# husheng876/pytorch_nested-unet

Hardware: AMD Instinct MI355X
Metric: images/sec NestedUNet 96x96 bs=16 train (higher is better)
Workload: dtype bf16; 1 GPU; NestedUNet(num_classes=1, in=3, deep_supervision=False) 96x96 per-GPU batch 16, bf16 storage / fp32 accumulate, BCEDiceLoss, SGD(1e-3, 0.9, wd 1e-4), fwd+loss+iou+bwd+sgd per step (BASELINE.json configs[1]); global_batch=16, parallelism=dp1, hip_graph=True

## Files before the change

include/nunet.h:

```cpp
#ifndef NUNET_H
#define NUNET_H

#include <stddef.h>
#include <stdint.h>

#ifdef __cplusplus
extern "C" {
#endif

typedef void* nunet_stream_t;

enum { NUNET_F32 = 0, NUNET_BF16 = 1, NUNET_F16 = 2 };
enum {
  NUNET_OK = 0,
  NUNET_EINVAL = -1,
  NUNET_ELAUNCH = -2,
  NUNET_ENODEV = -3
};

int nunet_version(void);
const char* nunet_last_error(void);

#define NUNET_BN_SUM_REPLICAS 8
#define NUNET_FX_WORDS 2

enum { NUNET_TF_NONE = 0, NUNET_TF_BN_RELU = 1, NUNET_TF_BN_RELU_BWD = 2 };

typedef struct {
  int32_t dtype;
  int32_t N, H, W;
  const void* src0; int32_t C0, P0;
  const void* src1; int32_t C1, P1;
  const void* wpack;
  const float* bias;
  void* dst0; int32_t D0, Q0;
  void* dst1; int32_t D1, Q1;
  int32_t acc_slot_w;
  uint32_t acc0_mask;
  int32_t acc1;
  int64_t* stats;
  float* splitk_ws;
  int64_t splitk_ws_floats;
  const void* bn_y; int32_t bn_py;
  const float* bn_mean_invstd;
  const float* bn_gamma; const float* bn_beta;
  int64_t* bn_sums;
  int32_t in_tf;
  int32_t tf_training;
  const void* tf_y; int32_t tf_py;
  const int64_t* tf_fx;
  const float* tf_gamma; const float* tf_beta; const float* tf_conv_bias;
  float* tf_running_mean; float* tf_running_var; int64_t* tf_nbt;
  float* tf_mean_invstd;
  float tf_momentum, tf_eps;
  float* tf_dgamma; float* tf_dbeta; float* tf_dbias;
  void* tf_store; int32_t tf_ps;
  int32_t tile;
} nunet_conv_desc;

int nunet_conv3x3_fwd(const nunet_conv_desc* d, nunet_stream_t s);

typedef struct {
  int32_t dtype;
  int32_t N, H, W;
  const void* src0; int32_t C0, P0;
  const void* src1; int32_t C1, P1;
  const void* dy;   int32_t Cout, PY;
  float* dw;
  int64_t slab_stride;
  int32_t max_slabs;
  int32_t target_wgs;
  int64_t dw_floats;
  int32_t item_shape;
} nunet_wgrad_desc;

int32_t nunet_conv3x3_wgrad_slabs(const nunet_wgrad_desc* d);
int nunet_conv3x3_wgrad(const nunet_wgrad_desc* d, nunet_stream_t s);
int nunet_conv3x3_wgrad_pair(const nunet_wgrad_desc* a, const nunet_wgrad_desc* b, nunet_stream_t stream);
int nunet_wgrad_reduce(const float* slabs, int64_t slab_stride, int32_t nslabs, int64_t n, float* out,
                       int32_t accumulate, nunet_stream_t s);

int nunet_pack_weights(const float* w_oihw, int32_t cout, int32_t cin, int32_t cin_pad,
                       int32_t dtype, void* wf, void* wd, nunet_stream_t s);
int nunet_unpack_wgrad(const float* dw, int32_t cout, int32_t cin, int32_t cin_pad,
                       float* g_oihw, int32_t accumulate, nunet_stream_t s);

typedef struct {
  int32_t dtype;
  int32_t N, H, W, C;
  const void* y; int32_t PY;
// ... 195 lines not shown
```

pytorch_nested-unet_amd/_lib.py:

```python
import ctypes as C
import os
import subprocess

import torch

_HERE = os.path.dirname(os.path.abspath(__file__))
LIB_PATH = os.environ.get("NUNET_LIB_PATH") or os.path.join(_HERE, "libnunet.so")

F32, BF16, F16 = 0, 1, 2
DTYPES = {"fp32": F32, "float32": F32, "bf16": BF16, "bfloat16": BF16, "fp16": F16, "float16": F16,
          torch.float32: F32, torch.bfloat16: BF16, torch.float16: F16}
TORCH_DTYPE = {F32: torch.float32, BF16: torch.bfloat16, F16: torch.float16}

_vp, _i32, _i64, _u32, _f32, _sz = C.c_void_p, C.c_int32, C.c_int64, C.c_uint32, C.c_float, C.c_size_t
BN_SUM_REPLICAS = 8
FX_WORDS = 2
TF_NONE, TF_BN_RELU, TF_BN_RELU_BWD = 0, 1, 2


def fx_zeros(c, device):
    return torch.zeros(BN_SUM_REPLICAS * 2 * c * FX_WORDS, dtype=torch.int64, device=device)


def fx_decode(buf, c):
    w = buf.detach().cpu().view(BN_SUM_REPLICAS, 2 * c, FX_WORDS).sum(0)
    return w[:, 0].double() * 2.0 ** -20 + w[:, 1].double() * 2.0 ** -60


def fx_encode(values, c, device):
    v = values.detach().cpu().double().reshape(2 * c) * 2.0 ** 20
    hi = torch.floor(v)
    lo = torch.floor((v - hi) * 2.0 ** 40)
    buf = torch.zeros(BN_SUM_REPLICAS, 2 * c, FX_WORDS, dtype=torch.int64)
    buf[0, :, 0] = hi.to(torch.int64)
    buf[0, :, 1] = lo.to(torch.int64)
    return buf.reshape(-1).to(device)


class ConvDesc(C.Structure):
    _fields_ = [("dtype", _i32), ("N", _i32), ("H", _i32), ("W", _i32),
                ("src0", _vp), ("C0", _i32), ("P0", _i32),
                ("src1", _vp), ("C1", _i32), ("P1", _i32),
                ("wpack", _vp), ("bias", _vp),
                ("dst0", _vp), ("D0", _i32), ("Q0", _i32),
                ("dst1", _vp), ("D1", _i32), ("Q1", _i32),
                ("acc_slot_w", _i32), ("acc0_mask", _u32), ("acc1", _i32),
                ("stats", _vp), ("splitk_ws", _vp), ("splitk_ws_floats", _i64),
                ("bn_y", _vp), ("bn_py", _i32), ("bn_mean_invstd", _vp), ("bn_gamma", _vp), ("bn_beta", _vp), ("bn_sums", _vp),
                ("in_tf", _i32), ("tf_training", _i32), ("tf_y", _vp), ("tf_py", _i32), ("tf_fx", _vp),
                ("tf_gamma", _vp), ("tf_beta", _vp), ("tf_conv_bias", _vp),
                ("tf_running_mean", _vp), ("tf_running_var", _vp), ("tf_nbt", _vp), ("tf_mean_invstd", _vp),
                ("tf_momentum", _f32), ("tf_eps", _f32),
                ("tf_dgamma", _vp), ("tf_dbeta", _vp), ("tf_dbias", _vp), ("tf_store", _vp), ("tf_ps", _i32), ("tile", _i32)]


class WgradDesc(C.Structure):
    _fields_ = [("dtype", _i32), ("N", _i32), ("H", _i32), ("W", _i32),
                ("src0", _vp), ("C0", _i32), ("P0", _i32),
                ("src1", _vp), ("C1", _i32), ("P1", _i32),
                ("dy", _vp), ("Cout", _i32), ("PY", _i32),
                ("dw", _vp), ("slab_stride", _i64), ("max_slabs", _i32), ("target_wgs", _i32), ("dw_floats", _i64), ("item_shape", _i32)]


class BnFwdDesc(C.Structure):
    _fields_ = [("dtype", _i32), ("N", _i32), ("H", _i32), ("W", _i32), ("C", _i32),
                ("y", _vp), ("PY", _i32),
                ("conv_bias", _vp), ("stats", _vp), ("gamma", _vp), ("beta", _vp),
                ("running_mean", _vp), ("running_var", _vp), ("num_batches_tracked", _vp),
                ("save_mean_invstd", _vp),
                ("training", _i32), ("momentum", _f32), ("eps", _f32),
                ("a", _vp), ("PA", _i32), ("pooled", _vp), ("PP", _i32), ("up", _vp), ("PU", _i32)]


class BnBwdDesc(C.Structure):
    _fields_ = [("dtype", _i32), ("N", _i32), ("H", _i32), ("W", _i32), ("C", _i32),
                ("da", _vp), ("PDA", _i32), ("y", _vp), ("PY", _i32),
                ("mean_invstd", _vp), ("gamma", _vp), ("beta", _vp),
                ("sums", _vp), ("dgamma", _vp), ("dbeta", _vp), ("dbias", _vp),
                ("dy", _vp), ("PDY", _i32)]


class BnrDesc(C.Structure):
    _fields_ = [("y", _vp), ("PY", _i32), ("mean_invstd", _vp), ("gamma", _vp), ("beta", _vp), ("sums", _vp)]


class ProfEntry(C.Structure):
# ... 180 lines not shown
```

pytorch_nested-unet_amd/csrc/conv3x3.hip:

```cpp
#include <stdlib.h>
#include <type_traits>

#include "common.h"

template <typename T> struct Mma;
template <> struct Mma<bf16_t> {
  typedef bf16x8 Frag;
  static __device__ __forceinline__ Frag load(const bf16_t* p) { return *reinterpret_cast<const bf16x8*>(p); }
  static __device__ __forceinline__ void mma(f32x16& acc, const Frag& a, const Frag& b) {
    acc = __builtin_amdgcn_mfma_f32_32x32x16_bf16(a, b, acc, 0, 0, 0);
  }
  static __device__ __forceinline__ void sink(const Frag& a) { asm volatile("" :: "v"(a)); }
};
template <> struct Mma<f16_t> {
  typedef f16x8 Frag;
  static __device__ __forceinline__ Frag load(const f16_t* p) { return *reinterpret_cast<const f16x8*>(p); }
  static __device__ __forceinline__ void mma(f32x16& acc, const Frag& a, const Frag& b) {
    acc = __builtin_amdgcn_mfma_f32_32x32x16_f16(a, b, acc, 0, 0, 0);
  }
  static __device__ __forceinline__ void sink(const Frag& a) { asm volatile("" :: "v"(a)); }
};
template <> struct Mma<float> {
  struct Frag { f32x4 lo, hi; };
  static __device__ __forceinline__ Frag load(const float* p) {
// ... 28 lines not shown
}

__host__ __device__ __forceinline__ unsigned fastdiv_inv(int d) { return d > 1 ? (unsigned)(((1ull << 32) + (unsigned)d - 1) / (unsigned)d) : 0u; }
__device__ __forceinline__ int fastdiv(int n, unsigned inv) { return inv ? (int)__umulhi((unsigned)n, inv) : n; }

template <bool ST>
__device__ __forceinline__ int map_pixel_t(int n, int y, int x, int N, int H, int W, int SH, unsigned SHinv) {
  if constexpr (ST) {
    const int yc = y < 0 ? 0 : y;
    const int n2 = (int)__umulhi((unsigned)yc, SHinv), yy = yc - n2 * SH - 1;
    const bool ok = (y >= 0) & (x >= 0) & (x < W) & (n2 < N) & (yy >= 0);
    const int gp = (n2 * H + yy) * W + x;
    return ok ? gp : -1;
  } else {
    const bool ok = (n < N) & (y >= 0) & (y < H) & (x >= 0) & (x < W);
    const int gp = (n * H + y) * W + x;
    return ok ? gp : -1;
  }
}

__device__ __attribute__((aligned(64))) uint32_t g_zero_page[2048 + 16];

struct ConvP {
  const void* src0; const void* src1;
  int C0, C1, P0, P1;
  const void* w; const float* bias;
  void* dst0; void* dst1;
  int D0, D1, Q0, Q1;
  int slot_w; unsigned acc0_mask; int acc1;
  unsigned inv_slot_w;
  long long* stats;
  int N, H, W, Cin, Cout;
  int NI, TH, TW, tilesX, tilesY, tilesG, nCoT, nItems;
  int SH;
  unsigned SHinv;
  unsigned invS, invCoT, invTX, invTY;
  unsigned invTHW, invTW, invHH2HW2, invHW2;
  int S, nch0, nch;
  float* slabs;
  long long slab_stride;
  const void* bn_y; int bn_py;
  const float* bn_mi; const float* bn_gamma; const float* bn_beta;
  long long* bn_sums;
  const void* tf_y; int tf_py;
  const long long* tf_fx;
  const float* tf_gamma; const float* tf_beta; const float* tf_bias;
  float* tf_rm; float* tf_rv; long long* tf_nbt;
  float* tf_save;
  int tf_training; float tf_momentum, tf_eps;
  float* tf_dgamma; float* tf_dbeta; float* tf_dbias;
  void* tf_store; int tf_ps;
  float M;
};

template <typename T, int WM_, int WN_, int SM_, int SN_> struct ConvCfg {
  static constexpr int WM = WM_, WN = WN_, SM = SM_, SN = SN_;
  static constexpr int NT = 64 * WM * WN;
  static constexpr int BM = 32 * SM * WM;
  static constexpr int BN = 32 * SN * WN;
  static constexpr int EPV = Tr<T>::EPV;
  static constexpr int KC = 64 / (int)sizeof(T);
  static constexpr int KS = KC / 16;
  static constexpr int PS = KC + EPV;
  static constexpr int HPMAX = (SM * SN == 4) ? 344 : BM + BM / 2;
  static constexpr int UH = (HPMAX * 4 + NT - 1) / NT;
  static constexpr int UW = (9 * BN * 4 + NT - 1) / NT;
  static constexpr int OS = BN + EPV;
  static constexpr int UO = (BM * (BN / EPV) + NT - 1) / NT;
  static constexpr int HALO_ELEMS = HPMAX * PS;
  static constexpr int W_ELEMS = 9 * BN * PS;
  static constexpr int STAGE_ELEMS = (HALO_ELEMS + W_ELEMS) > BM * OS ? (HALO_ELEMS + W_ELEMS) : BM * OS;
};

#ifdef NUNET_KSTAMP
__device__ unsigned long long* g_kstamp; __device__ int g_kstamp_wgs;
extern "C" int nunet_kstamp_set(void* buf, int wgs) {
  if (hipMemcpyToSymbol(HIP_SYMBOL(g_kstamp), &buf, sizeof(buf)) != hipSuccess) return 1;
  return hipMemcpyToSymbol(HIP_SYMBOL(g_kstamp_wgs), &wgs, sizeof(wgs)) != hipSuccess;
}
#define KSTAMP(i) do { if (threadIdx.x == 0 && (int)blockIdx.x < g_kstamp_wgs && (i) < 30) g_kstamp[blockIdx.x * 32 + (i)] = __builtin_amdgcn_s_memtime(); } while (0)
#define KSTAMP_RT(i) do { if (threadIdx.x == 0 && (int)blockIdx.x < g_kstamp_wgs) g_kstamp[blockIdx.x * 32 + (i)] = __builtin_amdgcn_s_memrealtime(); } while (0)
#else
#define KSTAMP(i) do {} while (0)
#define KSTAMP_RT(i) do {} while (0)
#endif

#ifndef NUNET_ABLATE
#define NUNET_ABLATE 0
#endif

static inline int conv_coef_floats(int lt, int cin, bool bnr, int cout) { return (lt == 1 ? 2 : lt == 2 ? 4 : 0) * cin + (bnr ? 4 * cout : 0) + cout; }

struct ConvGroup { int n; int grid[CONV_GROUP_MAX]; ConvP p[CONV_GROUP_MAX]; };

#ifndef NUNET_XCD_REMAP
#define NUNET_XCD_REMAP 1
#endif
__device__ __forceinline__ int xcd_remap(int b, int G) {
  if (!NUNET_XCD_REMAP) return b;
  const int x = b & 7, l = b >> 3, q = G >> 3, rem = G & 7;
  return (x < rem ? x * (q + 1) : rem * (q + 1) + (x - rem) * q) + l;
}
__device__ __forceinline__ void conv_group_decode(const ConvGroup& g, int b, int& k, int& v) {
  int base = 0, prevg = 0, live = g.n;
  k = 0; v = b;
#pragma unroll
  for (int j = 0; j < CONV_GROUP_MAX; ++j) {
    if (j < g.n) {
      const int span = (g.grid[j] - prevg) * live;
      if (b >= base && b < base + span) { const int r = b - base; const int q = r / live; k = j + (r - q * live); v = prevg + q; }
      base += span; prevg = g.grid[j]; --live;
    }
  }
}

template <typename T, int WM, int WN, int SM, int SN, bool SK, bool BNR, int LT>
__global__ __launch_bounds__(64 * WM * WN, 2) void conv3x3_kernel(ConvGroup grp) {
  typedef ConvCfg<T, WM, WN, SM, SN> C;
  int gk = 0, vbid = (int)blockIdx.x;
  if (grp.n > 1) conv_group_decode(grp, (int)blockIdx.x, gk, vbid);
  gk = __builtin_amdgcn_readfirstlane(gk); vbid = __builtin_amdgcn_readfirstlane(vbid);
  const ConvP& p = grp.p[gk];
  const int vgrid = grp.grid[gk];
  typedef Mma<T> M;
  constexpr int PS = C::PS, EPV = C::EPV, BN = C::BN, BM = C::BM, NT = C::NT, KS = C::KS, OS = C::OS;

  __shared__ __attribute__((aligned(16))) T s_buf[C::STAGE_ELEMS];
  __shared__ int s_hidx[BM];
  __shared__ int s_mxy[BM];
  __shared__ int s_hxy[C::HPMAX];
  __shared__ int s_gpix[BM];
  __shared__ float s_red[2 * WM * BN];
  extern __shared__ __attribute__((aligned(16))) float s_coef[];
  T* const s_halo = s_buf;
  T* const s_w = s_buf + C::HALO_ELEMS;
  float* const s_bnc = s_coef + (LT == 1 ? 2 : LT == 2 ? 4 : 0) * p.Cin;
  float* const s_bias = s_bnc + (BNR ? 4 : 0) * p.Cout;

  const int tid = threadIdx.x, lane = tid & 63, wave = tid >> 6;
  const int wm = wave / WN, wn = wave % WN;
  const int r = lane & 31, h = lane >> 5;
  const int HW2 = p.TW + 2, HH2 = p.TH + 2;
  const int HP = p.NI * HH2 * HW2;
  const int THW = p.TH * p.TW;
  KSTAMP(0); KSTAMP_RT(30);
  [[maybe_unused]] int kst = 4;

  for (int m = tid; m < BM; m += NT) {
    const int r32 = m & 31;
    const int q = (r32 < 4) ? r32 : (r32 < 12) ? r32 + 12 : (r32 < 16) ? r32 - 8 : (r32 < 20) ? r32 + 8 : (r32 < 28) ? r32 - 12 : r32;
    const int t = (m & ~31) + q;
    const int ni = fastdiv(t, p.invTHW);
    const int rem = t - ni * THW;
    const int ly = fastdiv(rem, p.invTW), lx = rem - ly * p.TW;
    const bool ok = ni < p.NI;
    s_hidx[m] = ok ? ((ni * HH2 + ly + 1) * HW2 + lx + 1) : (HW2 + 1);
    s_mxy[m] = ok ? ((ni << 20) | (ly << 10) | lx) : -1;
  }
  for (int hp = tid; hp < C::HPMAX; hp += NT) {
    int code = -1;
    if (hp < HP) {
      const int ni = fastdiv(hp, p.invHH2HW2);
      const int rem = hp - ni * (HH2 * HW2);
      const int hy = fastdiv(rem, p.invHW2), hx = rem - hy * HW2;
      code = (ni << 20) | (hy << 10) | hx;
    }
    s_hxy[hp] = code;
  }
// ... 58 lines not shown
    const int row = u >> 2;
    const int tap = row / BN, co = row - tap * BN;
    woff[k] = row < 9 * BN ? (unsigned)(((tap * p.Cout + co) * p.Cin + seg * EPV) * (int)sizeof(T)) : (unsigned)(seg * 16);
  }
  unsigned wco = 0u;
  auto set_ptrs = [&](const Item& it) { wco = (unsigned)(it.co0 * p.Cin * (int)sizeof(T)); };
  struct LoadCtx { const char* base; unsigned pb, cb, yb, ycb, wb; };
  auto load_ctx = [&](int kb) {
    LoadCtx c;
    const bool s0 = LT != 0 || kb < p.C0;
    c.base = (const char*)(s0 ? p.src0 : p.src1);
    c.pb = (unsigned)(s0 ? p.P0 : p.P1) * (unsigned)sizeof(T);
    c.cb = (unsigned)((s0 ? kb : kb - p.C0) * (int)sizeof(T) + seg * 16);
    c.yb = (unsigned)p.tf_py * (unsigned)sizeof(T);
    c.ycb = (unsigned)(kb * (int)sizeof(T) + seg * 16);
    c.wb = (unsigned)(kb * (int)sizeof(T)) + wco;
    return c;
  };
  constexpr int NU = C::UH + C::UW;
  auto load_unit = [&](const LoadCtx& c, int u) {
    if (u < C::UH) {
      const unsigned gp = hgp[u] < 0 ? 0u : (unsigned)hgp[u];
      hreg[u].raw = *reinterpret_cast<const u32x4*>(c.base + (gp * c.pb + c.cb));
      if constexpr (LT == 2) yreg[u].raw = *reinterpret_cast<const u32x4*>((const char*)p.tf_y + (gp * c.yb + c.ycb));
    } else {
      wreg[u - C::UH].raw = *reinterpret_cast<const u32x4*>((const char*)p.w + (woff[u - C::UH] + c.wb));
    }
  };
  auto load_regs = [&](int kb) {
    const LoadCtx c = load_ctx(kb);
#pragma unroll
    for (int u = 0; u < NU; ++u) load_unit(c, u);
  };
  auto write_lds = [&](int kb, bool store) {
    if constexpr (LT == 0) {
#pragma unroll
      for (int k = 0; k < C::UH; ++k) {
        const int u = tid + k * NT;
        if ((k + 1) * NT <= C::HPMAX * 4 || (u >> 2) < C::HPMAX) st16(&s_halo[(u >> 2) * PS + seg * EPV], hgp[k] >= 0 ? hreg[k] : zero16<T>());
      }
    } else {
      typedef typename FV<T>::type V;
      const int c0 = kb + seg * EPV;
      const V sc = ldf<T>(&s_coef[c0]), sh = ldf<T>(&s_coef[p.Cin + c0]);
      V cA, cB;
      if constexpr (LT == 2) { cA = ldf<T>(&s_coef[2 * p.Cin + c0]); cB = ldf<T>(&s_coef[3 * p.Cin + c0]); }
#pragma unroll
      for (int k = 0; k < C::UH; ++k) {
        const int u = tid + k * NT;
        if ((k + 1) * NT <= C::HPMAX * 4 || (u >> 2) < C::HPMAX) {
          const bool ok = hgp[k] >= 0;
          V v;
          if constexpr (LT == 1) v = bn_relu_apply<V>(vec_to_f<T>(hreg[k]), sc, sh);
          else v = bn_relu_bwd_apply<V>(vec_to_f<T>(hreg[k]), vec_to_f<T>(yreg[k]), sc, sh, cA, cB);
          Vec16<T> o = vec_from_f<T>(v);
          if (!ok) o = zero16<T>();
          st16(&s_halo[(u >> 2) * PS + seg * EPV], o);
          if (store && ok && ((interior >> k) & 1u)) st16((T*)p.tf_store + (size_t)hgp[k] * p.tf_ps + c0, o);
        }
      }
    }
#pragma unroll
    for (int k = 0; k < C::UW; ++k) {
      const int u = tid + k * NT;
      if ((k + 1) * NT <= 9 * BN * 4 || (u >> 2) < 9 * BN) st16(&s_w[(u >> 2) * PS + seg * EPV], wreg[k]);
    }
  };

  f32x16 acc[SM][SN];
#pragma unroll
  for (int a = 0; a < SM; ++a)
#pragma unroll
    for (int b = 0; b < SN; ++b)
#pragma unroll
      for (int i = 0; i < 16; ++i) acc[a][b][i] = 0.f;

  auto chunk_kb = [&](int c) { return c < p.nch0 ? c * C::KC : p.C0 + (c - p.nch0) * C::KC; };
  constexpr int NSTEP = 9 * KS;
  auto sweep = [&](auto LOADS, const LoadCtx& lc) {
    constexpr bool WITH_LOADS = decltype(LOADS)::value;
    constexpr int PD = 1;
    constexpr int NB = PD + 1;
    typename M::Frag fa[NB][SM], fb[NB][SN];
    auto read_step = [&](int j) {
      const int tap = j / KS, ks = j % KS, bu = j % NB;
#pragma unroll
      for (int a = 0; a < SM; ++a) fa[bu][a] = M::load(&s_halo[abase[a] + toff[tap] + ks * 16]);
#pragma unroll
      for (int b = 0; b < SN; ++b) fb[bu][b] = M::load(&s_w[bbase + (tap * BN + b * 32) * PS + ks * 16]);
    };
#pragma unroll
    for (int j = 0; j < PD; ++j) read_step(j);
#pragma unroll
    for (int j = 0; j < NSTEP; ++j) {
      if (j + PD < NSTEP && !(NUNET_ABLATE & 2)) read_step(j + PD);
      if constexpr (WITH_LOADS && !(NUNET_ABLATE & 4)) {
#pragma unroll
        for (int u = 0; u < NU; ++u)
          if ((u * NSTEP) / NU == j) load_unit(lc, u);
      }
      __builtin_amdgcn_sched_barrier(0);
#pragma unroll
      for (int a = 0; a < SM; ++a)
#pragma unroll
        for (int b = 0; b < SN; ++b) {
          if constexpr (NUNET_ABLATE & 1) { M::sink(fa[j % NB][a]); M::sink(fb[j % NB][b]); }
          else M::mma(acc[a][b], fa[j % NB][a], fb[j % NB][b]);
        }
      __builtin_amdgcn_sched_barrier(0);
    }
  };
  auto epi_sk = [&](const Item& cur) {
    float* slab = p.slabs + (size_t)cur.ks * p.slab_stride;
#pragma unroll
    for (int b = 0; b < SN; ++b) {
      const int co = cur.co0 + (wn * SN + b) * 32 + r;
#pragma unroll
      for (int a = 0; a < SM; ++a) {
#pragma unroll
        for (int i = 0; i < 16; ++i) {
          const int gp = s_gpix[(wm * SM + a) * 32 + acc_row(i, h)];
          if (gp >= 0) slab[(size_t)gp * p.Cout + co] = acc[a][b][i];
          acc[a][b][i] = 0.f;
        }
      }
    }
  };
  static_assert(SM * 16 <= 64, "row-validity mask of the epilogue is one 64-bit word");
  Vec16<T> byv[BNR ? C::UO : 1];
  auto issue_byv = [&](const Item& cur) {
    if constexpr (BNR) {
      constexpr int SEGS = BN / EPV;
// ... 66 lines not shown
    Vec16<T> vv[C::UO];
#pragma unroll
    for (int k = 0; k < C::UO; ++k) {
      const int m = m0 + k * (NT / SEGS);
      vv[k] = ld16(&s_out[(m < BM ? m : 0) * OS + sg * EPV]);
    }
#pragma unroll
    for (int k = 0; k < C::UO; ++k) {
      if (gpu[k] >= 0) {
        T* const q = qb + (size_t)gpu[k] * qs;
        Vec16<T> v = vv[k];
        if (any_accum && accum) v = vec_from_f<T>(vec_to_f<T>(v) + vec_to_f<T>(ld16(q)));
        if (!(NUNET_ABLATE & 64)) st16(q, v); else asm volatile("" :: "v"(v.raw));
        if constexpr (BNR && !(NUNET_ABLATE & 256)) {
          const V yf = vec_to_f<T>(byv[k]);
          const V dz = __builtin_elementwise_fma(yf, bsc, bsh) > V(0.f) ? vec_to_f<T>(v) : V(0.f);
          r1 += dz;
          r2 += dz * ((yf - bmean) * bistd);
        }
      }
    }
    KSTAMP(kst); ++kst;
    if constexpr (BNR && !(NUNET_ABLATE & 512)) {
#pragma unroll
      for (int off = SEGS; off < 64; off <<= 1) {
#pragma unroll
        for (int e = 0; e < EPV; ++e) {
          if (off == 4) { r1[e] += dpp_row_ror<4>(r1[e]); r2[e] += dpp_row_ror<4>(r2[e]); }
          else if (off == 8) { r1[e] += dpp_row_ror<8>(r1[e]); r2[e] += dpp_row_ror<8>(r2[e]); }
          else { r1[e] += __shfl_xor(r1[e], off); r2[e] += __shfl_xor(r2[e], off); }
        }
      }
      __syncthreads();
      float* s_bn = reinterpret_cast<float*>(s_buf);
      if (lane < SEGS) {
#pragma unroll
        for (int e = 0; e < EPV; ++e) {
          s_bn[(wave * 2 + 0) * BN + lane * EPV + e] = r1[e];
          s_bn[(wave * 2 + 1) * BN + lane * EPV + e] = r2[e];
        }
      }
      __syncthreads();
      for (int t = tid; t < 2 * BN; t += NT) {
        const int vsel = t / BN, c = t - vsel * BN;
        float sum = 0.f;
#pragma unroll
        for (int wv = 0; wv < WM * WN; ++wv) sum += s_bn[(wv * 2 + vsel) * BN + c];
        if (!(NUNET_ABLATE & 32)) fx_add(p.bn_sums + ((size_t)((vbid & (bn_sum_replicas(p.Cout) - 1)) * 2 + vsel) * p.Cout + cur.co0 + c) * NUNET_FX_WORDS, sum); else asm volatile("" :: "v"(sum));
      }
    }
    if (p.stats) {
      for (int t = tid; t < 2 * BN; t += NT) {
        const int vsel = t / BN, c = t - vsel * BN;
        float sum = 0.f;
#pragma unroll
        for (int k = 0; k < WM; ++k) sum += s_red[(k * BN + c) * 2 + vsel];
        if (!(NUNET_ABLATE & 32)) fx_add(p.stats + ((size_t)((vbid & (bn_sum_replicas(p.Cout) - 1)) * 2 + vsel) * p.Cout + cur.co0 + c) * NUNET_FX_WORDS, sum); else asm volatile("" :: "v"(sum));
      }
    }
  };
  int item = grp.n == 1 ? xcd_remap(vbid, vgrid) : vbid;
  if (item >= p.nItems) return;
  Item cur = decode(item);
  set_hgp(cur);
  set_ptrs(cur);
  int cc = 0, c_hi = 0;
  int kb = 0;
  if constexpr (SK) { cc = cur.ks * p.nch / p.S; c_hi = (cur.ks + 1) * p.nch / p.S; kb = chunk_kb(cc); }
  KSTAMP(2);
  load_regs(kb);
  bool first_chunk = true;
  for (int c = tid; c < p.Cout; c += NT) s_bias[c] = p.bias ? p.bias[c] : 0.f;
  if constexpr (BNR) {
    for (int c = tid; c < p.Cout; c += NT) {
      const float mean = p.bn_mi[c], istd = p.bn_mi[p.Cout + c];
      const float sc = p.bn_gamma[c] * istd;
      s_bnc[c] = mean; s_bnc[p.Cout + c] = istd; s_bnc[2 * p.Cout + c] = sc; s_bnc[3 * p.Cout + c] = __builtin_fmaf(-mean, sc, p.bn_beta[c]);
    }
  }
  if constexpr (LT == 1) {
    BnStatArgs a; a.fx = p.tf_fx; a.conv_bias = p.tf_bias; a.rm = p.tf_rm; a.rv = p.tf_rv; a.C = p.Cin; a.training = p.tf_training; a.M = p.M; a.eps = p.tf_eps;
    for (int c = tid; c < p.Cin; c += NT) {
      float mean, invstd, var, mf;
      bn_stat_coeffs(a, c, mean, invstd, var, mf);
      const float sc = p.tf_gamma[c] * invstd;
      s_coef[c] = sc; s_coef[p.Cin + c] = __builtin_fmaf(-mean, sc, p.tf_beta[c]);
      if (vbid == 0 && p.tf_training) {
        if (p.tf_save) { p.tf_save[c] = mean; p.tf_save[p.Cin + c] = invstd; }
        if (p.tf_rm) bn_running_update(p.tf_rm, p.tf_rv, c, p.tf_momentum, mf, var, p.M);
      }
    }
    if (vbid == 0 && p.tf_training && tid == 0 && p.tf_nbt) *p.tf_nbt += 1;
  }
  if constexpr (LT == 2) {
    const int nrep = bn_sum_replicas(p.Cin);
    for (int c = tid; c < p.Cin; c += NT) {
      const float mean = p.tf_save[c], istd = p.tf_save[p.Cin + c];
      const float sc = p.tf_gamma[c] * istd;
      double t1, t2;
      fx_totals(p.tf_fx, p.Cin, nrep, c, t1, t2);
      float A, B;
      bn_bwd_AB(mean, istd, sc, (float)(t1 / (double)p.M), (float)(t2 / (double)p.M), A, B);
      s_coef[c] = sc; s_coef[p.Cin + c] = __builtin_fmaf(-mean, sc, p.tf_beta[c]); s_coef[2 * p.Cin + c] = A; s_coef[3 * p.Cin + c] = B;
      if (vbid == 0) {
        if (p.tf_dbeta) p.tf_dbeta[c] = (float)t1;
        if (p.tf_dgamma) p.tf_dgamma[c] = (float)t2;
        if (p.tf_dbias) p.tf_dbias[c] = 0.f;
      }
    }
  }

  KSTAMP(3);
  while (true) {
    __syncthreads();
    KSTAMP(kst); ++kst;
    if (!(NUNET_ABLATE & 8) || (item == vbid && first_chunk)) write_lds(kb, LT != 0 && p.tf_store != nullptr && cur.co0 == 0);
    KSTAMP(kst); ++kst;
    if (first_chunk) {
      for (int m = tid; m < BM; m += NT) {
        const int code = s_mxy[m];
        int gp = -1;
        if (code >= 0) {
          const int n = cur.n0 + (code >> 20), y = cur.y0 + ((code >> 10) & 1023), x = cur.x0 + (code & 1023);
          gp = map_pixel(n, y, x, p.N, p.H, p.W, p.SH, p.SHinv);
        }
        s_gpix[m] = gp;
      }
    }
    __syncthreads();
    KSTAMP(kst); ++kst;
    int nkb = kb + C::KC, nitem = item, ncc = cc + 1, nc_hi = c_hi;
    Item nxt = cur;
    bool have_next = true;
    bool last_chunk;
    if constexpr (SK) last_chunk = ncc >= c_hi; else last_chunk = nkb >= p.Cin;
    if (last_chunk) {
      nkb = 0;
      nitem = item + vgrid;
      if (nitem < p.nItems) {
        nxt = decode(nitem); set_hgp(nxt); set_ptrs(nxt);
        if constexpr (SK) { ncc = nxt.ks * p.nch / p.S; nc_hi = (nxt.ks + 1) * p.nch / p.S; }
      } else have_next = false;
    }
    if (have_next) {
      if constexpr (SK) nkb = chunk_kb(ncc);
    }
    const LoadCtx lc = load_ctx(nkb);
    if constexpr (BNR && !SK && !(NUNET_ABLATE & 128)) { if (last_chunk) issue_byv(cur); }
    KSTAMP(kst); ++kst;
    if (have_next) sweep(std::true_type{}, lc); else sweep(std::false_type{}, lc);
    KSTAMP(kst); ++kst;
    first_chunk = false;
    if (last_chunk) {
      if constexpr (NUNET_ABLATE & 16) {
#pragma unroll
        for (int a = 0; a < SM; ++a)
#pragma unroll
          for (int b = 0; b < SN; ++b) asm volatile("" : "+v"(acc[a][b]));
      } else if constexpr (SK) epi_sk(cur); else epi_plain(cur, s_buf);
      KSTAMP(kst); ++kst;
      if (!have_next) { KSTAMP_RT(31); break; }
      cur = nxt; item = nitem; first_chunk = true;
    }
    kb = nkb; cc = ncc; c_hi = nc_hi;
  }
}

struct SplitFinP {
  const float* slabs; long long slab_stride; int S; const float* bias;
  void* dst0; void* dst1; int D0, D1, Q0, Q1; int slot_w; unsigned acc0_mask; int acc1; unsigned inv_slot_w;
  long long* stats; long long npix; int Cout;
  const void* bn_y; int bn_py; const float* bn_mi; const float* bn_gamma; const float* bn_beta; long long* bn_sums;
};
template <typename T, bool BNR>
__global__ __launch_bounds__(256) void splitk_finalize_kernel(SplitFinP p) {
  constexpr int EPV = Tr<T>::EPV;
  constexpr int NV = BNR ? 4 : 2;
  __shared__ float s_part[256 * NV * EPV];
  const int G = p.Cout / EPV;
  const int cg = threadIdx.x % G, co = cg * EPV;
  const int ppb = blockDim.x / G, pl = threadIdx.x / G;
  float q1[EPV], q2[EPV], r1[BNR ? EPV : 1], r2[BNR ? EPV : 1];
  float bmean[BNR ? EPV : 1], bistd[BNR ? EPV : 1], bsc[BNR ? EPV : 1], bsh[BNR ? EPV : 1], bias[EPV];
#pragma unroll
  for (int e = 0; e < EPV; ++e) {
    q1[e] = 0.f; q2[e] = 0.f;
    bias[e] = p.bias ? p.bias[co + e] : 0.f;
    if constexpr (BNR) {
      const int c = co + e;
      const float mean = p.bn_mi[c], istd = p.bn_mi[p.Cout + c];
      const float sc = p.bn_gamma[c] * istd;
      bmean[e] = mean; bistd[e] = istd; bsc[e] = sc; bsh[e] = __builtin_fmaf(-mean, sc, p.bn_beta[c]);
      r1[e] = 0.f; r2[e] = 0.f;
    }
  }
// ... 62 lines not shown
  TileGeom best{1, 1, 1, W, H, N, 0};
  double best_score = -1.0;
  for (int tw = 1; tw <= W && tw <= BM; ++tw) {
    for (int th = 1; th <= H && th * tw <= BM; ++th) {
      int nimax = (th == H && tw == W) ? BM / (H * W) : 1;
      if (nimax > N) nimax = N;
      for (int ni = 1; ni <= nimax; ++ni) {
        const long hp = (long)ni * (th + 2) * (tw + 2);
        if (hp > HPMAX) continue;
        const int tX = ceil_div(W, tw), tY = ceil_div(H, th), tG = ceil_div(N, ni);
        const double util = (double)N * H * W / ((double)tX * tY * tG * BM);
        const double halo = (double)hp / ((double)ni * th * tw);
        const double score = util * 1000.0 - halo * 10.0 + (tw >= 16 ? 1.0 : 0.0);
        if (score > best_score) { best_score = score; best = TileGeom{ni, th, tw, tX, tY, tG, 0}; }
      }
    }
  }
  if (W <= BM && (long)N * (H + 1) < (1 << 20) && H + 1 <= 4096) {
    const double best_util = (double)N * H * W / ((double)best.tilesX * best.tilesY * best.tilesG * BM);
    const int VH = N * (H + 1);
    double su = 0.0; int sth = 0;
    for (int th = 1; th * W <= BM && th < 1000; ++th) {
      if ((long)(th + 2) * (W + 2) > HPMAX) break;
      const int tY = ceil_div(VH, th);
      const double util = (double)N * H * W / ((double)tY * BM);
      if (util > su) { su = util; sth = th; }
    }
    if (sth > 0 && su > best_util * 1.08) best = TileGeom{1, sth, W, 1, ceil_div(VH, sth), 1, H + 1};
  }
  return best;
}

template <typename T, int WM, int WN, int SM, int SN, bool SK, bool BNR>
static void launch_conv_lt(int lt, unsigned grid, size_t dyn, hipStream_t st, const ConvGroup& g) {
  typedef ConvCfg<T, WM, WN, SM, SN> C;
  if (lt == 1) NUNET_LAUNCH((conv3x3_kernel<T, WM, WN, SM, SN, SK, BNR, 1>), dim3(grid), dim3(C::NT), dyn, st, g);
  else if (lt == 2) NUNET_LAUNCH((conv3x3_kernel<T, WM, WN, SM, SN, SK, BNR, 2>), dim3(grid), dim3(C::NT), dyn, st, g);
  else NUNET_LAUNCH((conv3x3_kernel<T, WM, WN, SM, SN, SK, BNR, 0>), dim3(grid), dim3(C::NT), dyn, st, g);
}

struct ConvSetup { ConvP p; long grid; size_t dyn; bool bnr; int lt; double flops, bytes; };
template <typename T, int WM, int WN, int SM, int SN>
static void conv_setup(const nunet_conv_desc* d, ConvSetup& S) {
  typedef ConvCfg<T, WM, WN, SM, SN> C;
  ConvP& p = S.p;
  p.src0 = d->src0; p.src1 = d->src1; p.C0 = d->C0; p.C1 = d->C1; p.P0 = d->P0; p.P1 = d->P1;
  p.w = d->wpack; p.bias = d->bias;
  p.dst0 = d->dst0; p.dst1 = d->dst1; p.D0 = d->D0; p.D1 = d->D1; p.Q0 = d->Q0; p.Q1 = d->Q1;
  p.slot_w = d->acc_slot_w; p.acc0_mask = d->acc0_mask; p.acc1 = d->acc1; p.inv_slot_w = fastdiv_inv(d->acc_slot_w);
  p.stats = (long long*)d->stats;
  p.N = d->N; p.H = d->H; p.W = d->W; p.Cin = d->C0 + d->C1; p.Cout = d->D0 + d->D1;
  p.M = (float)d->N * d->H * d->W;
  const bool bnr = d->bn_y != nullptr;
  const int lt = d->in_tf;
  p.bn_y = d->bn_y; p.bn_py = d->bn_py; p.bn_mi = d->bn_mean_invstd; p.bn_gamma = d->bn_gamma; p.bn_beta = d->bn_beta; p.bn_sums = (long long*)d->bn_sums;
  p.tf_y = d->tf_y; p.tf_py = d->tf_py; p.tf_fx = (const long long*)d->tf_fx; p.tf_gamma = d->tf_gamma; p.tf_beta = d->tf_beta; p.tf_bias = d->tf_conv_bias;
  p.tf_rm = d->tf_running_mean; p.tf_rv = d->tf_running_var; p.tf_nbt = (long long*)d->tf_nbt; p.tf_save = d->tf_mean_invstd;
  p.tf_training = d->tf_training; p.tf_momentum = d->tf_momentum; p.tf_eps = d->tf_eps;
  p.tf_dgamma = d->tf_dgamma; p.tf_dbeta = d->tf_dbeta; p.tf_dbias = d->tf_dbias; p.tf_store = d->tf_store; p.tf_ps = d->tf_ps;
  const TileGeom g = nunet_choose_tile(d->N, d->H, d->W, C::BM, C::HPMAX);
  p.NI = g.NI; p.TH = g.TH; p.TW = g.TW; p.tilesX = g.tilesX; p.tilesY = g.tilesY; p.tilesG = g.tilesG; p.SH = g.SH;
  p.SHinv = g.SH ? (unsigned)(((1ull << 32) + g.SH - 1) / g.SH) : 0u;
  p.nCoT = p.Cout / C::BN;
  long items = (long)p.nCoT * g.tilesX * g.tilesY * g.tilesG;
  p.S = 1; p.slabs = nullptr; p.slab_stride = 0;
  p.nch0 = p.C0 / C::KC;
  p.nch = p.nch0 + p.C1 / C::KC;
#ifndef NUNET_SK_ITEMS
#define NUNET_SK_ITEMS 60
#define NUNET_SK_TARGET 320
#endif
  if (d->splitk_ws && items <= NUNET_SK_ITEMS && p.nch >= 8 && p.Cout <= 1024 && (256 / (p.Cout / C::EPV)) >= 1) {
    int Sn = (int)((NUNET_SK_TARGET + items - 1) / items);
    if (Sn > p.nch / 2) Sn = p.nch / 2;
    const long long need = (long long)Sn * d->N * d->H * d->W * p.Cout;
    if (Sn > 1 && need <= d->splitk_ws_floats) {
      p.S = Sn; p.slabs = d->splitk_ws; p.slab_stride = (long long)d->N * d->H * d->W * p.Cout;
      items *= Sn;
    }
  }
  p.nItems = (int)items;
  p.invS = fastdiv_inv(p.S); p.invCoT = fastdiv_inv(p.nCoT); p.invTX = fastdiv_inv(p.tilesX); p.invTY = fastdiv_inv(p.tilesY);
  p.invTHW = fastdiv_inv(g.TH * g.TW); p.invTW = fastdiv_inv(g.TW); p.invHH2HW2 = fastdiv_inv((g.TH + 2) * (g.TW + 2)); p.invHW2 = fastdiv_inv(g.TW + 2);
  S.bnr = bnr; S.lt = lt;
  S.dyn = sizeof(float) * (size_t)conv_coef_floats(lt, p.Cin, bnr && p.S == 1, p.Cout);
  const size_t lds_bytes = sizeof(T) * C::STAGE_ELEMS + 4 * (3 * C::BM + C::HPMAX) + 8 * WM * C::BN + S.dyn;
  long per_cu = (long)(160 * 1024 / lds_bytes);
  if (per_cu < 1) per_cu = 1;
  if (per_cu > 2048 / C::NT) per_cu = 2048 / C::NT;
  const long resident = 256 * per_cu;
  const long rounds = (items + resident - 1) / resident;
  S.grid = (items + rounds - 1) / rounds;
  const double px = (double)d->N * d->H * d->W;
  const int acin = g_prof_alg_cin > 0 ? g_prof_alg_cin : p.Cin;
  S.flops = 2.0 * 9 * acin * p.Cout * px;
  S.bytes = (px * (acin * (lt == 2 ? 2 : 1) + p.Cout) + 9.0 * acin * p.Cout) * sizeof(T);
}

template <typename T, int WM, int WN, int SM, int SN>
static int launch_conv_cfg(const nunet_conv_desc* const* ds, int n, hipStream_t st) {
  typedef ConvCfg<T, WM, WN, SM, SN> C;
  ConvSetup S[CONV_GROUP_MAX];
  for (int k = 0; k < n; ++k) conv_setup<T, WM, WN, SM, SN>(ds[k], S[k]);
  const int cls = C::BN == 64 ? PC_CONV_M128N64 : C::BM == 256 ? PC_CONV_M256N32 : PC_CONV_M128N32;
  if (n == 1 && S[0].p.S > 1) {
    const ConvSetup& s0 = S[0];
    const ConvP& p = s0.p;
    const nunet_conv_desc* d = ds[0];
    ProfScope ps(cls, s0.flops, s0.bytes, st);
    ConvGroup g; g.n = 1; g.grid[0] = (int)s0.grid; g.p[0] = p;
    launch_conv_lt<T, WM, WN, SM, SN, true, false>(s0.lt, (unsigned)s0.grid, s0.dyn, st, g);
    SplitFinP f;
    f.slabs = p.slabs; f.slab_stride = p.slab_stride; f.S = p.S; f.bias = p.bias;
    f.dst0 = p.dst0; f.dst1 = p.dst1; f.D0 = p.D0; f.D1 = p.D1; f.Q0 = p.Q0; f.Q1 = p.Q1;
    f.slot_w = p.slot_w; f.acc0_mask = p.acc0_mask; f.acc1 = p.acc1; f.inv_slot_w = p.inv_slot_w; f.stats = p.stats;
    f.npix = (long long)d->N * d->H * d->W; f.Cout = p.Cout;
    f.bn_y = p.bn_y; f.bn_py = p.bn_py; f.bn_mi = p.bn_mi; f.bn_gamma = p.bn_gamma; f.bn_beta = p.bn_beta; f.bn_sums = p.bn_sums;
    const int G = p.Cout / C::EPV;
    const int blk = G * (256 / G);
    long long fg = (f.npix + (blk / G) - 1) / (blk / G);
    if (fg > 1024) fg = 1024;
    if (s0.bnr) NUNET_LAUNCH((splitk_finalize_kernel<T, true>), dim3((unsigned)fg), dim3(blk), 0, st, f);
    else NUNET_LAUNCH((splitk_finalize_kernel<T, false>), dim3((unsigned)fg), dim3(blk), 0, st, f);
    return nunet_check_launch("conv3x3 (K-split)");
  }
  int order[CONV_GROUP_MAX];
  for (int k = 0; k < n; ++k) order[k] = k;
  for (int a = 0; a < n; ++a) for (int b = a + 1; b < n; ++b) if (S[order[b]].grid < S[order[a]].grid) { const int t = order[a]; order[a] = order[b]; order[b] = t; }
  ConvGroup g; g.n = n;
  long total = 0; size_t dyn = 0; double fl = 0, by = 0;
  for (int k = 0; k < n; ++k) {
    const ConvSetup& s = S[order[k]];
    g.grid[k] = (int)s.grid; g.p[k] = s.p; total += s.grid; if (s.dyn > dyn) dyn = s.dyn; fl += s.flops; by += s.bytes;
  }
  ProfScope ps(cls, fl, by, st);
  if (S[0].bnr) launch_conv_lt<T, WM, WN, SM, SN, false, true>(S[0].lt, (unsigned)total, dyn, st, g);
  else launch_conv_lt<T, WM, WN, SM, SN, false, false>(S[0].lt, (unsigned)total, dyn, st, g);
  return nunet_check_launch(n > 1 ? "conv3x3 (group)" : "conv3x3");
}

static int conv_cfg_of(const nunet_conv_desc* d) {
  const int cout = d->D0 + d->D1;
  if (d->tile >= 1 && d->tile <= 4) return d->tile - 1;
  const long px = (long)d->N * d->H * d->W;
  const long items_std = cout % 64 == 0 ? ceil_div64(px, 128) * (cout / 64) : ceil_div64(px, 256) * (cout / 32);
  const bool small = items_std < 256 || (cout == 32 && d->in_tf != NUNET_TF_BN_RELU_BWD && px < (1L << 20)) ||
                     (cout == 64 && d->in_tf != NUNET_TF_BN_RELU_BWD && px < (1L << 16));
  if (small) return 0;
  return cout % 64 == 0 ? 1 : 2;
}
template <typename T> static int launch_conv_n(const nunet_conv_desc* const* ds, int n, hipStream_t st) {
  const int cfg = conv_cfg_of(ds[0]);
  if (cfg == 0) return launch_conv_cfg<T, 4, 1, 1, 1>(ds, n, st);
  if (cfg == 1) return launch_conv_cfg<T, 2, 2, 2, 1>(ds, n, st);
  if (cfg == 3) return launch_conv_cfg<T, 4, 1, 2, 2>(ds, n, st);
  return launch_conv_cfg<T, 4, 1, 2, 1>(ds, n, st);
}
template <typename T> static int launch_conv(const nunet_conv_desc* d, hipStream_t st) { return launch_conv_n<T>(&d, 1, st); }

template <typename T> static int conv_is_split(const nunet_conv_desc* d) {
  ConvSetup S;
  const int cfg = conv_cfg_of(d);
  if (cfg == 0) conv_setup<T, 4, 1, 1, 1>(d, S); else if (cfg == 1) conv_setup<T, 2, 2, 2, 1>(d, S); else if (cfg == 3) conv_setup<T, 4, 1, 2, 2>(d, S); else conv_setup<T, 4, 1, 2, 1>(d, S);
  return S.p.S > 1 ? 1 : 0;
}

static int conv_check(const nunet_conv_desc* d);
int nunet_conv_group_key(const nunet_conv_desc* d) {
  if (!d || conv_check(d) != NUNET_OK) return -1;
  if (NUNET_DISPATCH(d->dtype, conv_is_split, d)) return -1;
  return ((d->dtype * 4 + conv_cfg_of(d)) * 2 + (d->bn_y ? 1 : 0)) * 3 + d->in_tf;
}
int nunet_conv3x3_group(const nunet_conv_desc* const* ds, int n, hipStream_t st) {
  NUNET_REQUIRE(ds && n >= 1 && n <= CONV_GROUP_MAX, "conv3x3 group: 1..%d problems", CONV_GROUP_MAX);
  const int key = nunet_conv_group_key(ds[0]);
  for (int k = 0; k < n; ++k) { const int rc = conv_check(ds[k]); if (rc) return rc; }
  if (n > 1) for (int k = 0; k < n; ++k) NUNET_REQUIRE(key >= 0 && nunet_conv_group_key(ds[k]) == key, "conv3x3 group: problems of different kernel variants");
  return NUNET_DISPATCH(ds[0]->dtype, launch_conv_n, ds, n, st);
}

static int conv_check(const nunet_conv_desc* d) {
  NUNET_REQUIRE(d && d->src0 && d->wpack && d->dst0, "conv3x3: null pointer");
  const int cin = d->C0 + d->C1, cout = d->D0 + d->D1;
  NUNET_REQUIRE(d->dtype >= 0 && d->dtype <= 2, "conv3x3: bad dtype %d", d->dtype);
  const int kc = 64 / dtype_size(d->dtype);
  NUNET_REQUIRE(d->N > 0 && d->H > 0 && d->W > 0, "conv3x3: bad extent %dx%dx%d", d->N, d->H, d->W);
  NUNET_REQUIRE(d->C0 > 0 && d->C0 % kc == 0 && d->C1 % kc == 0, "conv3x3: C0=%d C1=%d must be multiples of %d (64-byte channel chunks)", d->C0, d->C1, kc);
  NUNET_REQUIRE(d->C1 == 0 || d->src1, "conv3x3: src1 null with C1=%d", d->C1);
  NUNET_REQUIRE(cout % 32 == 0 && d->D0 % 32 == 0 && d->D1 % 32 == 0, "conv3x3: D0=%d D1=%d must be multiples of 32", d->D0, d->D1);
  NUNET_REQUIRE(d->D1 == 0 || d->dst1, "conv3x3: dst1 null with D1=%d", d->D1);
  NUNET_REQUIRE(d->P0 >= d->C0 && (d->C1 == 0 || d->P1 >= d->C1) && d->Q0 >= d->D0 && (d->D1 == 0 || d->Q1 >= d->D1), "conv3x3: pitch smaller than channels");
  const int epv = 16 / dtype_size(d->dtype);
  NUNET_REQUIRE(d->P0 % epv == 0 && (d->C1 == 0 || d->P1 % epv == 0), "conv3x3: source pitch must keep 16-byte alignment");
  NUNET_REQUIRE(d->acc_slot_w == 0 || d->acc_slot_w % 32 == 0, "conv3x3: acc_slot_w %d", d->acc_slot_w);
  {
    const unsigned long long px = (unsigned long long)d->N * d->H * d->W, es = dtype_size(d->dtype);
    const unsigned long long lim = 1ull << 32;
    NUNET_REQUIRE(px < (1ull << 30) && px * d->P0 * es < lim && (d->C1 == 0 || px * d->P1 * es < lim) && 9ull * cout * cin * es < lim &&
                  (d->in_tf != 2 || px * d->tf_py * es < lim), "conv3x3: problem too large (every input tensor must span < 4 GB)");
  }
  if (d->bn_y) {
    NUNET_REQUIRE(d->bn_mean_invstd && d->bn_gamma && d->bn_beta && d->bn_sums, "conv3x3: fused BN-backward reduce needs mean/invstd, gamma, beta and sums");
    NUNET_REQUIRE(d->D1 == 0 && d->Q0 == d->D0 && d->acc0_mask == 0 && d->bn_py % epv == 0 && cout <= 512,
                  "conv3x3: fused BN-backward reduce needs one dense, assign-only destination");
  }
  NUNET_REQUIRE(d->in_tf >= 0 && d->in_tf <= 2, "conv3x3: in_tf %d", d->in_tf);
  NUNET_REQUIRE(d->tile >= 0 && d->tile <= 4 && ((d->tile != 2 && d->tile != 4) || cout % 64 == 0), "conv3x3: tile %d with Cout=%d", d->tile, cout);
  if (d->in_tf) {
    NUNET_REQUIRE(d->C1 == 0 && cin <= 1024, "conv3x3: an input transform needs a single source (C1 == 0) of at most 1024 channels");
    NUNET_REQUIRE(d->tf_gamma && d->tf_beta, "conv3x3: input transform needs gamma and beta");
    NUNET_REQUIRE(!d->tf_store || d->tf_ps % epv == 0, "conv3x3: tf_store pitch alignment");
    if (d->in_tf == 1) {
      if (d->tf_training) NUNET_REQUIRE(d->tf_fx, "conv3x3: BN input transform in training mode needs the producing conv's sums");
      else NUNET_REQUIRE(d->tf_running_mean && d->tf_running_var, "conv3x3: BN input transform in eval mode needs running statistics");
    } else {
      NUNET_REQUIRE(d->tf_y && d->tf_fx && d->tf_mean_invstd && d->tf_py % epv == 0, "conv3x3: BN-backward input transform needs y, sums and saved mean/invstd");
    }
  }
  return NUNET_OK;
}
extern "C" int nunet_conv3x3_fwd(const nunet_conv_desc* d, nunet_stream_t s) {
  const int rc = conv_check(d);
  if (rc) return rc;
  return NUNET_DISPATCH(d->dtype, launch_conv, d, (hipStream_t)s);
}

struct WgP {
  const void* src0; const void* src1;
  int C0, C1, P0, P1;
  const void* dy; int Cout, PY;
  float* dw; long long slab_stride;
  int N, H, W, Cin;
  int NI, TH, TW, tilesX, tilesY, tilesG;
  int nCoT, nCiT, ksplit, nMT;
  int SH; unsigned SHinv;
  unsigned invTX, invTY;
};

template <typename T, int A_, int B_> struct WgCfg {
  static constexpr int A = A_, B = B_;
// ... 441 lines not shown
```

Before: 9621 images/sec.

## Reuse LDS input halo across output-channel tiles in BN-backward conv walk

```diff
diff --git a/include/nunet.h b/include/nunet.h
--- a/include/nunet.h
+++ b/include/nunet.h
@@ -56,6 +56,7 @@
   float* tf_dgamma; float* tf_dbeta; float* tf_dbias;
   void* tf_store; int32_t tf_ps;
   int32_t tile;
+  int32_t halo_reuse;
 } nunet_conv_desc;
 
 int nunet_conv3x3_fwd(const nunet_conv_desc* d, nunet_stream_t s);
diff --git a/pytorch_nested-unet_amd/_lib.py b/pytorch_nested-unet_amd/_lib.py
--- a/pytorch_nested-unet_amd/_lib.py
+++ b/pytorch_nested-unet_amd/_lib.py
@@ -51,7 +51,8 @@
                 ("tf_gamma", _vp), ("tf_beta", _vp), ("tf_conv_bias", _vp),
                 ("tf_running_mean", _vp), ("tf_running_var", _vp), ("tf_nbt", _vp), ("tf_mean_invstd", _vp),
                 ("tf_momentum", _f32), ("tf_eps", _f32),
-                ("tf_dgamma", _vp), ("tf_dbeta", _vp), ("tf_dbias", _vp), ("tf_store", _vp), ("tf_ps", _i32), ("tile", _i32)]
+                ("tf_dgamma", _vp), ("tf_dbeta", _vp), ("tf_dbias", _vp), ("tf_store", _vp), ("tf_ps", _i32), ("tile", _i32),
+                ("halo_reuse", _i32)]
 
 
 class WgradDesc(C.Structure):
diff --git a/pytorch_nested-unet_amd/csrc/conv3x3.hip b/pytorch_nested-unet_amd/csrc/conv3x3.hip
--- a/pytorch_nested-unet_amd/csrc/conv3x3.hip
+++ b/pytorch_nested-unet_amd/csrc/conv3x3.hip
@@ -84,6 +84,7 @@
   long long* stats;
   int N, H, W, Cin, Cout;
   int NI, TH, TW, tilesX, tilesY, tilesG, nCoT, nItems;
+  int run;
   int SH;
   unsigned SHinv;
   unsigned invS, invCoT, invTX, invTY;
@@ -122,6 +123,7 @@
   static constexpr int HALO_ELEMS = HPMAX * PS;
   static constexpr int W_ELEMS = 9 * BN * PS;
   static constexpr int STAGE_ELEMS = (HALO_ELEMS + W_ELEMS) > BM * OS ? (HALO_ELEMS + W_ELEMS) : BM * OS;
+  static constexpr bool HALO_REUSE = sizeof(T) == 2 && BM * OS <= W_ELEMS;
 };
 
 #ifdef NUNET_KSTAMP
@@ -166,7 +168,7 @@
   }
 }
 
-template <typename T, int WM, int WN, int SM, int SN, bool SK, bool BNR, int LT>
+template <typename T, int WM, int WN, int SM, int SN, bool SK, bool BNR, int LT, bool RUN = false>
 __global__ __launch_bounds__(64 * WM * WN, 2) void conv3x3_kernel(ConvGroup grp) {
   typedef ConvCfg<T, WM, WN, SM, SN> C;
   int gk = 0, vbid = (int)blockIdx.x;
@@ -178,6 +180,9 @@
   constexpr int PS = C::PS, EPV = C::EPV, BN = C::BN, BM = C::BM, NT = C::NT, KS = C::KS, OS = C::OS;
 
   __shared__ __attribute__((aligned(16))) T s_buf[C::STAGE_ELEMS];
+  static_assert(!RUN || (LT == 2 && !SK && C::HALO_REUSE), "halo-reuse walk: BN-backward loader, no K-split, 16-bit types");
+  constexpr bool CAN_RUN = RUN;
+  constexpr bool run = RUN;
   __shared__ int s_hidx[BM];
   __shared__ int s_mxy[BM];
   __shared__ int s_hxy[C::HPMAX];
@@ -186,6 +191,7 @@
   extern __shared__ __attribute__((aligned(16))) float s_coef[];
   T* const s_halo = s_buf;
   T* const s_w = s_buf + C::HALO_ELEMS;
+  T* const s_out = CAN_RUN ? s_w : s_buf;
   float* const s_bnc = s_coef + (LT == 1 ? 2 : LT == 2 ? 4 : 0) * p.Cin;
   float* const s_bias = s_bnc + (BNR ? 4 : 0) * p.Cout;
 
@@ -310,8 +316,9 @@
 #pragma unroll
     for (int u = 0; u < NU; ++u) load_unit(c, u);
   };
-  auto write_lds = [&](int kb, bool store) {
-    if constexpr (LT == 0) {
+  auto write_lds = [&](int kb, bool store, bool halo) {
+    if (!halo) {
+    } else if constexpr (LT == 0) {
 #pragma unroll
       for (int k = 0; k < C::UH; ++k) {
         const int u = tid + k * NT;
@@ -356,7 +363,7 @@
   auto chunk_kb = [&](int c) { return c < p.nch0 ? c * C::KC : p.C0 + (c - p.nch0) * C::KC; };
   constexpr int NSTEP = 9 * KS;
   auto sweep = [&](auto LOADS, const LoadCtx& lc) {
-    constexpr bool WITH_LOADS = decltype(LOADS)::value;
+    constexpr int WITH_LOADS = decltype(LOADS)::value;
     constexpr int PD = 1;
     constexpr int NB = PD + 1;
     typename M::Frag fa[NB][SM], fb[NB][SN];
@@ -372,10 +379,10 @@
 #pragma unroll
     for (int j = 0; j < NSTEP; ++j) {
       if (j + PD < NSTEP && !(NUNET_ABLATE & 2)) read_step(j + PD);
-      if constexpr (WITH_LOADS && !(NUNET_ABLATE & 4)) {
+      if constexpr (WITH_LOADS > 0 && !(NUNET_ABLATE & 4)) {
 #pragma unroll
         for (int u = 0; u < NU; ++u)
-          if ((u * NSTEP) / NU == j) load_unit(lc, u);
+          if ((u * NSTEP) / NU == j && (WITH_LOADS == 2 || u >= C::UH)) load_unit(lc, u);
       }
       __builtin_amdgcn_sched_barrier(0);
 #pragma unroll
@@ -508,7 +515,7 @@
         }
       }
       __syncthreads();
-      float* s_bn = reinterpret_cast<float*>(s_buf);
+      float* s_bn = reinterpret_cast<float*>(s_out);
       if (lane < SEGS) {
 #pragma unroll
         for (int e = 0; e < EPV; ++e) {
@@ -536,7 +543,11 @@
     }
   };
   int item = grp.n == 1 ? xcd_remap(vbid, vgrid) : vbid;
-  if (item >= p.nItems) return;
+  int item_end = p.nItems, istep = vgrid;
+  if (run) { item *= p.run; item_end = min(item + p.run, p.nItems); istep = 1; }
+  if (item >= item_end) return;
+  const int item0 = item;
+  bool keep_halo = false;
   Item cur = decode(item);
   set_hgp(cur);
   set_ptrs(cur);
@@ -590,9 +601,9 @@
   while (true) {
     __syncthreads();
     KSTAMP(kst); ++kst;
-    if (!(NUNET_ABLATE & 8) || (item == vbid && first_chunk)) write_lds(kb, LT != 0 && p.tf_store != nullptr && cur.co0 == 0);
+    if (!(NUNET_ABLATE & 8) || (item == item0 && first_chunk)) write_lds(kb, LT != 0 && p.tf_store != nullptr && cur.co0 == 0, !keep_halo);
     KSTAMP(kst); ++kst;
-    if (first_chunk) {
+    if (first_chunk && !keep_halo) {
       for (int m = tid; m < BM; m += NT) {
         const int code = s_mxy[m];
         int gp = -1;
@@ -610,12 +621,14 @@
     bool have_next = true;
     bool last_chunk;
     if constexpr (SK) last_chunk = ncc >= c_hi; else last_chunk = nkb >= p.Cin;
+    bool next_keeps = false;
     if (last_chunk) {
       nkb = 0;
-      nitem = item + vgrid;
-      if (nitem < p.nItems) {
+      nitem = item + istep;
+      if (nitem < item_end) {
         nxt = decode(nitem); set_hgp(nxt); set_ptrs(nxt);
         if constexpr (SK) { ncc = nxt.ks * p.nch / p.S; nc_hi = (nxt.ks + 1) * p.nch / p.S; }
+        next_keeps = run && nxt.co0 != 0;
       } else have_next = false;
     }
     if (have_next) {
@@ -624,7 +637,9 @@
     const LoadCtx lc = load_ctx(nkb);
     if constexpr (BNR && !SK && !(NUNET_ABLATE & 128)) { if (last_chunk) issue_byv(cur); }
     KSTAMP(kst); ++kst;
-    if (have_next) sweep(std::true_type{}, lc); else sweep(std::false_type{}, lc);
+    if (!have_next) sweep(std::integral_constant<int, 0>{}, lc);
+    else if (CAN_RUN && next_keeps) { if constexpr (CAN_RUN) sweep(std::integral_constant<int, 1>{}, lc); }
+    else sweep(std::integral_constant<int, 2>{}, lc);
     KSTAMP(kst); ++kst;
     first_chunk = false;
     if (last_chunk) {
@@ -633,10 +648,10 @@
         for (int a = 0; a < SM; ++a)
 #pragma unroll
           for (int b = 0; b < SN; ++b) asm volatile("" : "+v"(acc[a][b]));
-      } else if constexpr (SK) epi_sk(cur); else epi_plain(cur, s_buf);
+      } else if constexpr (SK) epi_sk(cur); else epi_plain(cur, s_out);
       KSTAMP(kst); ++kst;
       if (!have_next) { KSTAMP_RT(31); break; }
-      cur = nxt; item = nitem; first_chunk = true;
+      cur = nxt; item = nitem; first_chunk = true; keep_halo = next_keeps;
     }
     kb = nkb; cc = ncc; c_hi = nc_hi;
   }
@@ -765,11 +780,19 @@
 }
 
 template <typename T, int WM, int WN, int SM, int SN, bool SK, bool BNR>
-static void launch_conv_lt(int lt, unsigned grid, size_t dyn, hipStream_t st, const ConvGroup& g) {
+static void launch_conv_lt(int lt, bool run, unsigned grid, size_t dyn, hipStream_t st, const ConvGroup& g) {
   typedef ConvCfg<T, WM, WN, SM, SN> C;
+  if constexpr (!SK && C::HALO_REUSE) {
+    if (lt == 2 && run) { NUNET_LAUNCH((conv3x3_kernel<T, WM, WN, SM, SN, false, BNR, 2, true>), dim3(grid), dim3(C::NT), dyn, st, g); return; }
+  }
   if (lt == 1) NUNET_LAUNCH((conv3x3_kernel<T, WM, WN, SM, SN, SK, BNR, 1>), dim3(grid), dim3(C::NT), dyn, st, g);
   else if (lt == 2) NUNET_LAUNCH((conv3x3_kernel<T, WM, WN, SM, SN, SK, BNR, 2>), dim3(grid), dim3(C::NT), dyn, st, g);
   else NUNET_LAUNCH((conv3x3_kernel<T, WM, WN, SM, SN, SK, BNR, 0>), dim3(grid), dim3(C::NT), dyn, st, g);
+}
+
+static bool conv_halo_reuse(const nunet_conv_desc* d, int lt, int S, int nch, int nCoT, bool fits) {
+  if (lt != NUNET_TF_BN_RELU_BWD || S != 1 || nch != 1 || nCoT < 2 || !fits) return false;
+  return d->halo_reuse != 1;
 }
 
 struct ConvSetup { ConvP p; long grid; size_t dyn; bool bnr; int lt; double flops, bytes; };
@@ -824,6 +847,8 @@
   const long resident = 256 * per_cu;
   const long rounds = (items + resident - 1) / resident;
   S.grid = (items + rounds - 1) / rounds;
+  p.run = 0;
+  if (conv_halo_reuse(d, lt, p.S, p.nch, p.nCoT, C::HALO_REUSE)) p.run = (int)rounds;
   const double px = (double)d->N * d->H * d->W;
   const int acin = g_prof_alg_cin > 0 ? g_prof_alg_cin : p.Cin;
   S.flops = 2.0 * 9 * acin * p.Cout * px;
@@ -842,7 +867,7 @@
     const nunet_conv_desc* d = ds[0];
     ProfScope ps(cls, s0.flops, s0.bytes, st);
     ConvGroup g; g.n = 1; g.grid[0] = (int)s0.grid; g.p[0] = p;
-    launch_conv_lt<T, WM, WN, SM, SN, true, false>(s0.lt, (unsigned)s0.grid, s0.dyn, st, g);
+    launch_conv_lt<T, WM, WN, SM, SN, true, false>(s0.lt, false, (unsigned)s0.grid, s0.dyn, st, g);
     SplitFinP f;
     f.slabs = p.slabs; f.slab_stride = p.slab_stride; f.S = p.S; f.bias = p.bias;
     f.dst0 = p.dst0; f.dst1 = p.dst1; f.D0 = p.D0; f.D1 = p.D1; f.Q0 = p.Q0; f.Q1 = p.Q1;
@@ -867,8 +892,9 @@
     g.grid[k] = (int)s.grid; g.p[k] = s.p; total += s.grid; if (s.dyn > dyn) dyn = s.dyn; fl += s.flops; by += s.bytes;
   }
   ProfScope ps(cls, fl, by, st);
-  if (S[0].bnr) launch_conv_lt<T, WM, WN, SM, SN, false, true>(S[0].lt, (unsigned)total, dyn, st, g);
-  else launch_conv_lt<T, WM, WN, SM, SN, false, false>(S[0].lt, (unsigned)total, dyn, st, g);
+  const bool run = S[0].p.run > 0;
+  if (S[0].bnr) launch_conv_lt<T, WM, WN, SM, SN, false, true>(S[0].lt, run, (unsigned)total, dyn, st, g);
+  else launch_conv_lt<T, WM, WN, SM, SN, false, false>(S[0].lt, run, (unsigned)total, dyn, st, g);
   return nunet_check_launch(n > 1 ? "conv3x3 (group)" : "conv3x3");
 }
 
@@ -891,18 +917,19 @@
 }
 template <typename T> static int launch_conv(const nunet_conv_desc* d, hipStream_t st) { return launch_conv_n<T>(&d, 1, st); }
 
-template <typename T> static int conv_is_split(const nunet_conv_desc* d) {
+template <typename T> static int conv_walk_of(const nunet_conv_desc* d) {
   ConvSetup S;
   const int cfg = conv_cfg_of(d);
   if (cfg == 0) conv_setup<T, 4, 1, 1, 1>(d, S); else if (cfg == 1) conv_setup<T, 2, 2, 2, 1>(d, S); else if (cfg == 3) conv_setup<T, 4, 1, 2, 2>(d, S); else conv_setup<T, 4, 1, 2, 1>(d, S);
-  return S.p.S > 1 ? 1 : 0;
+  return S.p.S > 1 ? 1 : S.p.run > 0 ? 2 : 0;
 }
 
 static int conv_check(const nunet_conv_desc* d);
 int nunet_conv_group_key(const nunet_conv_desc* d) {
   if (!d || conv_check(d) != NUNET_OK) return -1;
-  if (NUNET_DISPATCH(d->dtype, conv_is_split, d)) return -1;
-  return ((d->dtype * 4 + conv_cfg_of(d)) * 2 + (d->bn_y ? 1 : 0)) * 3 + d->in_tf;
+  const int walk = NUNET_DISPATCH(d->dtype, conv_walk_of, d);
+  if (walk == 1) return -1;
+  return (((d->dtype * 4 + conv_cfg_of(d)) * 2 + (d->bn_y ? 1 : 0)) * 3 + d->in_tf) * 2 + (walk == 2 ? 1 : 0);
 }
 int nunet_conv3x3_group(const nunet_conv_desc* const* ds, int n, hipStream_t st) {
   NUNET_REQUIRE(ds && n >= 1 && n <= CONV_GROUP_MAX, "conv3x3 group: 1..%d problems", CONV_GROUP_MAX);
@@ -939,6 +966,7 @@
   }
   NUNET_REQUIRE(d->in_tf >= 0 && d->in_tf <= 2, "conv3x3: in_tf %d", d->in_tf);
   NUNET_REQUIRE(d->tile >= 0 && d->tile <= 4 && ((d->tile != 2 && d->tile != 4) || cout % 64 == 0), "conv3x3: tile %d with Cout=%d", d->tile, cout);
+  NUNET_REQUIRE(d->halo_reuse >= 0 && d->halo_reuse <= 2, "conv3x3: halo_reuse %d", d->halo_reuse);
   if (d->in_tf) {
     NUNET_REQUIRE(d->C1 == 0 && cin <= 1024, "conv3x3: an input transform needs a single source (C1 == 0) of at most 1024 channels");
     NUNET_REQUIRE(d->tf_gamma && d->tf_beta, "conv3x3: input transform needs gamma and beta");
```

Result: no change. 9640 images/sec, median of 5 (+0.2%).
